# baaivision/Painter

Measured on AMD Instinct MI355X. Metric: images/sec (896x448 pairs) ViT-L fwd+bwd, higher is better.
Workload: dtype bf16; 1 GPU; painter_vit_large_patch16_input896x448 bf16 batch=8/GPU fwd+bwd on 1xMI355X (BASELINE configs[1]); global_batch=8, image=896x448x3 stitched pair, mode=train (DropPath 0.1), parallelism=dp1, rccl_ranks=0, backend=n/a, grad_allreduce=n/a

## Files before the change

include/painter_hip.h:

```cpp
#ifndef PAINTER_HIP_H
#define PAINTER_HIP_H

#include <stdint.h>

#ifdef __cplusplus
extern "C" {
#endif

#ifndef __HIP__
typedef struct ihipStream_t* hipStream_t;
#endif

enum { PA_F32 = 0, PA_BF16 = 1 };
enum {
    PA_EPI_BIAS = 0,
    PA_EPI_BIAS_F32 = 1,
    PA_EPI_BIAS_GELU = 2,
    PA_EPI_BIAS_RESID = 3
};

#define PA_ABI_VERSION 8
int pa_abi_version(void);
int pa_debug_set(int which, int value);
int pa_debug_get(int which);
// ... 5 lines not shown
int pa_linear_fwd_skip(int dtype, int epilogue, const void* x, int64_t ldx, const void* w, const float* bias, void* out, void* out2,
                       int64_t ldo, const float* resid, const float* rowscale, int rows_per_sample, int M, int N, int K,
                       const float* rowskip, int skip_rows_per_sample, hipStream_t stream);
int pa_linear_pixshuf(int dtype, const void* x, int64_t ldx, const void* w , const float* bias,
                      void* out_nhwc, int batch, int Hp, int Wp, int P, int C, int K, hipStream_t stream);
int64_t pa_linear_dgrad_workspace_bytes(int M, int K);
int pa_linear_dgrad(int dtype, const void* dy , int64_t lddy, const void* w ,
                    const void* gelu_aux , void* dx , int64_t lddx, float* dx_colsum,
                    void* workspace, int M, int N, int K, hipStream_t stream);
int pa_linear_dgrad_skip(int dtype, const void* dy, int64_t lddy, const void* w, const void* gelu_aux, void* dx, int64_t lddx, float* dx_colsum,
                         void* workspace, int M, int N, int K, const float* rowskip , int skip_rows_per_sample,
                         hipStream_t stream);
int64_t pa_linear_wgrad_workspace_bytes(int dtype, int M, int N, int K);
int pa_linear_wgrad(int dtype, const void* dy , int64_t lddy, const void* x , int64_t ldx,
                    float* dw , void* workspace, int M, int N, int K, hipStream_t stream);
int64_t pa_colsum_workspace_bytes(int M, int N);
int pa_colsum(int dtype, const void* x , int64_t ld, int M, int N, float* out , void* workspace,
              hipStream_t stream);
int pa_slab_reduce(const float* in, float* out, int64_t n, int nz, int64_t stride, int accumulate, hipStream_t stream);

int pa_layernorm_fwd(int dtype, const float* x, int64_t ldx, const float* gamma, const float* beta, float eps,
                     void* y , int64_t ldy, float* mean, float* rstd,
                     int R, int D, hipStream_t stream);
int64_t pa_layernorm_bwd_workspace_bytes(int R, int D);
int pa_layernorm_bwd(int dtype, const void* dy, int64_t lddy, const float* x, int64_t ldx, const float* mean,
                     const float* rstd, const float* gamma, const float* dres, float* dx, int64_t lddx, void* dxT,
                     int64_t lddxT, const float* rowscale, int rows_per_sample, float* dgamma_dbeta, float* dxT_colsum,
                     void* workspace, int R, int D, hipStream_t stream);
int pa_layernorm_bwd_reduce(const void* workspace, float* dgamma_dbeta, float* dxT_colsum, int with_colsum, int R, int D,
                            hipStream_t stream);
// ... 196 lines not shown
```

painter_amd/_lib.py:

```python
import ctypes
import os
import re

HERE = os.path.dirname(os.path.abspath(__file__))
HEADER = os.path.join(os.path.dirname(HERE), "include", "painter_hip.h")
LIB_PATH = os.environ.get("PAINTER_AMD_LIB") or os.path.join(HERE, "lib", "libpainter_hip.so")

PA_F32, PA_BF16 = 0, 1
EPI_BIAS, EPI_BIAS_F32, EPI_BIAS_GELU, EPI_BIAS_RESID = 0, 1, 2, 3
(KNOB_G256_STAGGER, KNOB_G256_NOSTORE, KNOB_G256_ORDER, KNOB_WGRAD_TARGET, KNOB_G256_SHORT_TILES, KNOB_G256_ILV, KNOB_RELPOS_SPLITS,
 KNOB_ATTN3_FUSE, KNOB_ATTN_LIGHT_LAST, KNOB_CONV_WGRAD_GROUPS, KNOB_LN_BWD_VARIANT, KNOB_G256_PATCH, KNOB_G256_MIXED) = range(13)
KNOB_G256_MIXED_NFULL, KNOB_DROP_SKIP, KNOB_DECODER_ROWS, KNOB_COUNT = 14, 16, 17, 18

_CT = {"int": ctypes.c_int, "int64_t": ctypes.c_int64, "float": ctypes.c_float, "hipStream_t": ctypes.c_void_p}


def parse_header(path=HEADER):
    src = open(path).read()
    src = re.sub(r"/\*.*?\*/", " ", src, flags=re.S)
    src = re.sub(r"//[^\n]*", " ", src)
    protos = {}
    for m in re.finditer(r"\b(int64_t|int)\s+(pa_\w+)\s*\(([^)]*)\)\s*;", src):
        ret, name, args = m.group(1), m.group(2), m.group(3).strip()
        argtypes = []
        if args and args != "void":
            for a in args.split(","):
                a = a.strip()
# ... 47 lines not shown
```

painter_amd/csrc/common.h:

```cpp
#pragma once
#include <hip/hip_runtime.h>
#include <stdint.h>
#include <cstdlib>

typedef __bf16 bf16;
typedef __attribute__((ext_vector_type(8))) __bf16 bf16x8;
typedef __attribute__((ext_vector_type(16))) float f32x16;

#define DEVI __device__ __forceinline__

template <typename T> struct TT;
template <> struct TT<float> {
    static constexpr int EPC = 4;
    static constexpr int BK = 32;
    static constexpr int KSTEPS = 2;
    static constexpr int SPF = 2;
    typedef uint4 Vec4;
};
template <> struct TT<bf16> {
    static constexpr int EPC = 8;
    static constexpr int BK = 64;
    static constexpr int KSTEPS = 4;
    static constexpr int SPF = 1;
    typedef uint2 Vec4;
// ... 69 lines not shown

enum Knob {
    KNOB_G256_STAGGER = 0,
    KNOB_G256_NOSTORE = 1,
    KNOB_G256_ORDER = 2,
    KNOB_WGRAD_TARGET = 3,
    KNOB_G256_SHORT_TILES = 4,
    KNOB_G256_ILV = 5,
    KNOB_RELPOS_SPLITS = 6,
    KNOB_ATTN3_FUSE = 7,
    KNOB_ATTN_LIGHT_LAST = 8,
    KNOB_CONV_WGRAD_GROUPS = 9,
    KNOB_LN_BWD_VARIANT = 10,
    KNOB_G256_PATCH = 11,
    KNOB_G256_MIXED = 12,
    KNOB_FREE_13 = 13,
    KNOB_G256_MIXED_NFULL = 14,
    KNOB_FREE_15 = 15,
    KNOB_DROP_SKIP = 16,
    KNOB_DECODER_ROWS = 17,
    KNOB_COUNT = 18
};
inline int g_knob[KNOB_COUNT] = {};
static inline bool drop_skip_on() {
    static const int env = [] { const char* v = getenv("PAINTER_AMD_DROP_SKIP"); return v ? atoi(v) : 1; }();
    return g_knob[KNOB_DROP_SKIP] == 1 ? false : (g_knob[KNOB_DROP_SKIP] == 2 ? true : env != 0);
}
static inline bool decoder_rows_on() {
    static const int env = [] { const char* v = getenv("PAINTER_AMD_DECODER_ROWS"); return v ? atoi(v) : 1; }();
    return g_knob[KNOB_DECODER_ROWS] == 1 ? false : (g_knob[KNOB_DECODER_ROWS] == 2 ? true : env != 0);
}

inline long long g_attn_counts[6] = {0, 0, 0, 0, 0, 0};

DEVI float gelu_f(float x) { return 0.5f * x * (1.0f + erff(x * 0.70710678118654752f)); }
DEVI float gelu_grad_f(float x) {
    const float cdf = 0.5f * (1.0f + erff(x * 0.70710678118654752f));
    const float pdf = 0.39894228040143268f * __expf(-0.5f * x * x);
    return cdf + x * pdf;
}

// ... 71 lines not shown
```

painter_amd/csrc/gemm.hip:

```cpp
#include <cstdlib>
#include "gemm_engine.h"
#include "gemm256.h"
#include "../../include/painter_hip.h"

template <typename OutT> struct EpiBias {
    OutT* out; size_t ldo; const float* bias; int M, N;
    DEVI void operator()(const f32x16 (&acc)[2][2], int ib, int jb, int lane, int) const {
        foreach_acc(acc, ib, jb, lane, [&](int i, int j, float v) {
            if (i < M && j < N) out[(size_t)i * ldo + j] = from_f<OutT>(v + (bias ? bias[j] : 0.f));
        });
    }
};
constexpr float G8_OFF = 0.13f, G8_SCALE = 255.f / 1.26f, G8_STEP = 1.26f / 255.f;
DEVI uint32_t g8_code(float g) { return min((uint32_t)fmaf(g, G8_SCALE, G8_OFF * G8_SCALE + 0.5f), 255u); }
DEVI float g8_value(uint32_t q) { return fmaf((float)q, G8_STEP, -G8_OFF); }
template <typename T> struct GeluAux { typedef T type; };
template <> struct GeluAux<bf16> { typedef unsigned char type; };
template <typename T> struct EpiBiasGelu {
    typename GeluAux<T>::type* aux; T* act; size_t ld; const float* bias; int M, N;
    DEVI void operator()(const f32x16 (&acc)[2][2], int ib, int jb, int lane, int) const {
        foreach_acc(acc, ib, jb, lane, [&](int i, int j, float v) {
            if (i < M && j < N) {
                const T p = from_f<T>(v + bias[j]);
                if constexpr (std::is_same<T, bf16>::value) {
// ... 487 lines not shown
                                    rowskip, skip_rows_per_sample);
    return linear_dgrad_t<float>((const float*)dy, lddy, (const float*)w, (const float*)gelu_aux, (float*)dx, lddx, dx_colsum, (float*)workspace, M, N, K, st);
}
extern "C" int pa_linear_dgrad(int dtype, const void* dy, int64_t lddy, const void* w, const void* gelu_aux,
                               void* dx, int64_t lddx, float* dx_colsum, void* workspace, int M, int N, int K, hipStream_t st) {
    return pa_linear_dgrad_skip(dtype, dy, lddy, w, gelu_aux, dx, lddx, dx_colsum, workspace, M, N, K, nullptr, 1, st);
}

static bool wgrad_fast(int dtype, int M, int N, int K) {
    return dtype == PA_BF16 && g256::ok(N, K, M, true, true, N, K) && K % 4 == 0 && N % 256 == 0 && K % 256 == 0;
}
static int wgrad_fast_splits(int M, int N, int K) {
    const int tiles = (N / 256) * (K / 256);
    static const int env_target = [] { const char* v = getenv("PA_WGRAD_WGS"); return v ? atoi(v) : 0; }();
    int target = env_target > 0 ? env_target : (g_knob[KNOB_WGRAD_TARGET] > 0 ? g_knob[KNOB_WGRAD_TARGET] : 256);
    if (target < 16) target = 16;
    int s = (target + 3 * tiles / 4) / tiles;
    if (s < 1) s = 1;
    const int ktiles = M / 64;
    if (s > ktiles / 4) s = ktiles / 4 > 0 ? ktiles / 4 : 1;
    return g256::splits_used(M, s);
}
static int wgrad_splits(int M, int N, int K, int bk) {
    const int tiles = ((N + 127) / 128) * ((K + 127) / 128);
    const int nku = (M + bk - 1) / bk;
    int s = (640 + tiles - 1) / tiles;
    if (s > nku) s = nku;
    if (s > 64) s = 64;
    if (s < 1) s = 1;
    return s;
}
extern "C" int64_t pa_linear_wgrad_workspace_bytes(int dtype, int M, int N, int K) {
    if (wgrad_fast(dtype, M, N, K)) {
        const int s = wgrad_fast_splits(M, N, K);
        return s > 1 ? (int64_t)s * N * K * sizeof(float) : 0;
    }
    const int s = wgrad_splits(M, N, K, dtype == PA_BF16 ? 64 : 32);
    return s > 1 ? (int64_t)s * N * K * sizeof(float) : 0;
}
template <typename T>
static int linear_wgrad_t(const T* dy, int64_t lddy, const T* x, int64_t ldx, float* dw, float* ws, int M, int N, int K,
                          hipStream_t st) {
    if constexpr (std::is_same<T, bf16>::value) {
        if (wgrad_fast(PA_BF16, M, N, K) && g256::ok(N, K, M, true, true, lddy, ldx)) {
            const int s = wgrad_fast_splits(M, N, K);
            if (s == 1) return g256::launch<true, true>(dy, lddy, x, ldx, Epi4Slab{dw, (size_t)K, 0, N, K}, N, K, M, 1, st);
            int e = g256::launch<true, true>(dy, lddy, x, ldx, Epi4Slab{ws, (size_t)K, (size_t)N * K, N, K}, N, K, M, s, st);
            if (e) return e;
            return pa_slab_reduce(ws, dw, (int64_t)N * K, s, (int64_t)N * K, 0, st);
        }
    }
    OpT<T> A{dy, (size_t)lddy, N, 0};
    OpT<T> B{x, (size_t)ldx, K, 0};
    const int s = wgrad_splits(M, N, K, TT<T>::BK);
    if (s == 1) return launch_gemm<T, 2, 2>(A, B, EpiSlab{dw, (size_t)K, 0, N, K}, N, K, M, 1, 1, st);
    int e = launch_gemm<T, 2, 2>(A, B, EpiSlab{ws, (size_t)K, (size_t)N * K, N, K}, N, K, M, s, 1, st);
    if (e) return e;
    return pa_slab_reduce(ws, dw, (int64_t)N * K, s, (int64_t)N * K, 0, st);
}
extern "C" int pa_linear_wgrad(int dtype, const void* dy, int64_t lddy, const void* x, int64_t ldx, float* dw,
                               void* workspace, int M, int N, int K, hipStream_t st) {
    if (N % 4 || K % 4) return (int)hipErrorInvalidValue;
    if (dtype == PA_BF16) return linear_wgrad_t<bf16>((const bf16*)dy, lddy, (const bf16*)x, ldx, dw, (float*)workspace, M, N, K, st);
    return linear_wgrad_t<float>((const float*)dy, lddy, (const float*)x, ldx, dw, (float*)workspace, M, N, K, st);
}

extern "C" int pa_fill_dead_rows(void* x, int64_t pitch_bytes, int64_t row_bytes, const int* rowmap, int M, hipStream_t st);
extern "C" int pa_linear_dgrad_live(const void* dy, int64_t lddy, const void* w, void* dx, int64_t lddx, const int* live, const int* rowmap,
                                    const int* count, int M, int N, int K, hipStream_t st) {
    if (live == nullptr || rowmap == nullptr || count == nullptr || M < 8 || K % 8 || lddx % 8) return (int)hipErrorInvalidValue;
    if (!g256::ok(M, K, N, false, true, lddy, K)) return (int)hipErrorInvalidValue;
    int e = pa_fill_dead_rows(dx, lddx * 2, (int64_t)K * 2, rowmap, M, st);
    if (e) return e;
    return g256::launch_live<false, true>((const bf16*)dy, lddy, (const bf16*)w, K, Epi4Scatter{(bf16*)dx, (size_t)lddx, live, count, M, K}, M, K, N, count, st);
}
extern "C" int pa_linear_wgrad_live(const void* dy, int64_t lddy, const void* x, int64_t ldx, float* dw, const int* count, int M, int N, int K,
                                    hipStream_t st) {
    if (count == nullptr || M < 128 || M % 128) return (int)hipErrorInvalidValue;
    if (!wgrad_fast(PA_BF16, M, N, K) || !g256::ok(N, K, M, true, true, lddy, ldx)) return (int)hipErrorInvalidValue;
// ... 13 lines not shown
```

painter_amd/csrc/gemm256.h:

```cpp
#pragma once
#include "common.h"
#include <cstdlib>
#include <type_traits>

namespace g256 {

constexpr int BM = 256, BN = 256, BK = 64, NT = 512;
constexpr int LDS_BYTES = 131072;
typedef __attribute__((address_space(3))) void lds_void;
typedef __attribute__((address_space(1))) const void gbl_cvoid;

DEVI constexpr int unit_off(bool isB, int sub, int stage) { return (isB ? 65536 : 0) + sub * 32768 + stage * 16384; }

template <int N> DEVI void wait_vm() { asm volatile("s_waitcnt vmcnt(%0)" ::"n"(N) : "memory"); }
DEVI void wait_lgkm0() { asm volatile("s_waitcnt lgkmcnt(0)" ::: "memory"); }

template <bool MM, bool IS_A>
DEVI uint32_t src_off(int tid, int j, int sub, int tile0, int rows, uint32_t ld) {
    const int cidx = j * NT + tid;
    if constexpr (!MM) {
        const int u = cidx >> 3, p = cidx & 7;
        const int kc = p ^ ((u >> 1) & 7);
        int row = IS_A ? ((u >> 6) * 128 + sub * 64 + (u & 63)) : ((u >> 5) * 64 + sub * 32 + (u & 31));
        row = min(tile0 + row, rows - 1);
        return ((uint32_t)row * ld + kc * 8) * 2u;
    } else {
        const int k = cidx >> 4, cp = cidx & 15;
        const int c = cp ^ (4 * (k & 3));
        int n = IS_A ? ((c >> 3) * 128 + sub * 64 + (c & 7) * 8) : ((c >> 2) * 64 + sub * 32 + (c & 3) * 8);
        n = min(tile0 + n, rows - 8);
        return ((uint32_t)k * ld + n) * 2u;
    }
}

DEVI const unsigned char* sgpr_ptr(const unsigned char* p) {
    asm volatile("" : "+s"(p));
    return p;
}
DEVI void dma16(const unsigned char* g, unsigned char* l) {
    __builtin_amdgcn_global_load_lds((gbl_cvoid*)g, (lds_void*)l, 16, 0, 0);
}

template <int OFF> DEVI void lds_read128(uint4& d, uint32_t addr) {
    asm volatile("ds_read_b128 %0, %1 offset:%2" : "=v"(d) : "v"(addr), "n"(OFF) : "memory");
}
template <int OFF> DEVI void lds_read64_tr(uint2& d, uint32_t addr) {
    asm volatile("ds_read_b64_tr_b16 %0, %1 offset:%2" : "=v"(d) : "v"(addr), "n"(OFF) : "memory");
}

template <bool MM> struct Frag4;
template <> struct Frag4<false> {
    uint4 q0, q1, q2, q3;
    template <int IMM> DEVI void read(const uint32_t (&base)[4], int) {
// ... 22 lines not shown
    template <int KS> DEVI bf16x8 k() const {
        typedef __attribute__((ext_vector_type(2))) uint32_t u2;
        typedef __attribute__((ext_vector_type(4))) uint32_t u4;
        const uint2 l = KS == 0 ? l0 : KS == 1 ? l1 : KS == 2 ? l2 : l3;
        const uint2 h = KS == 0 ? h0 : KS == 1 ? h1 : KS == 2 ? h2 : h3;
        u2 lv = {l.x, l.y}, hv = {h.x, h.y};
        return __builtin_bit_cast(bf16x8, __builtin_shufflevector(lv, hv, 0, 1, 2, 3));
    }
};

template <class Epi> struct epi_colsum { static constexpr bool value = false; };
template <class Epi, class = void> struct epi_hi_off { static constexpr int value = 4; };
template <class Epi> struct epi_hi_off<Epi, std::void_t<decltype(Epi::HI_OFF)>> { static constexpr int value = Epi::HI_OFF; };
constexpr int BM_SHORT = 224;
constexpr int BM_HALF = 128;
template <bool AMM, bool BMM, int ILV, class Epi, bool SHORT = false, bool MIXED = false, bool SKIP = false, bool LIVE = false>
__global__ __launch_bounds__(NT) void gemm256_kernel(const bf16* __restrict__ Ag, uint32_t lda, const bf16* __restrict__ Bg,
                                                      uint32_t ldb, Epi epi, int M, int N, int ktiles, int ktiles_per_split,
                                                      int tiles_n, int stagger, int order, int nfull, int patch,
                                                      const float* __restrict__ rowskip, int rps, const int* __restrict__ live_count) {
    static_assert(!(LIVE && (SHORT || MIXED || SKIP)), "a device-side count goes with uniform 256-row tiles");
    static_assert(!(SHORT && AMM), "the 224-row tile is built for a K-major A operand");
    static_assert(!(SKIP && AMM), "row tiles are skipped only for a K-major A operand");
    static_assert(!(MIXED && (AMM || SHORT)), "half tiles are built for a K-major A operand and 256-row full tiles");
    constexpr int BMR = SHORT ? BM_SHORT : BM;
    extern __shared__ __attribute__((aligned(1024))) unsigned char smem[];
    const int tid = threadIdx.x, lane = tid & 63;
    if (stagger > 0 && blockIdx.x < 256 && blockIdx.y == 0) {
        const int64_t wait = ((int64_t)stagger * (((blockIdx.x >> 3) * 5) & 15)) >> 4;
        const uint64_t t0 = __builtin_amdgcn_s_memtime();
        while ((int64_t)(__builtin_amdgcn_s_memtime() - t0) < wait) __builtin_amdgcn_s_sleep(16);
    }
    const int wv = __builtin_amdgcn_readfirstlane(tid >> 6);
    const int wr = wv >> 2, wc = wv & 3;

    const bool htile = MIXED && (int)blockIdx.x >= nfull * tiles_n;
    int nwg = MIXED ? (htile ? (int)gridDim.x - nfull * tiles_n : nfull * tiles_n) : (int)gridDim.x;
    if constexpr (LIVE) {
        if constexpr (AMM) {
// ... 70 lines not shown
        if (skipped) {
            const int d = bid - nwg;
            int r = d / tiles_n;
            tn = d - r * tiles_n;
            bool found = false;
            skipped_ranges([&](int a, int b) {
                if (!found && r < b - a) { tm = a + r; found = true; }
                if (!found) r -= b - a;
            });
        } else {
            skipped_ranges([&](int a, int b) { if (tm >= a) tm += b - a; });
        }
    }
    const int i0 = htile ? nfull * BMR + tm * BM_HALF : tm * BMR, j0 = tn * BN;
    const bool blk3 = !(SHORT && wr == 1);
    const int kt0 = split * ktiles_per_split;
    const int nt = min(ktiles - kt0, ktiles_per_split);
    const bool empty = LIVE && AMM && nt == 0;
    uint32_t oa[2][2], ob[2][2];
#pragma unroll
    for (int sub = 0; sub < 2; ++sub)
#pragma unroll
        for (int j = 0; j < 2; ++j) {
            oa[sub][j] = src_off<AMM, true>(tid, j, sub, i0, M, lda);
            ob[sub][j] = src_off<BMM, false>(tid, j, sub, j0, N, ldb);
        }
    const size_t a_step = AMM ? (size_t)BK * lda * 2 : (size_t)BK * 2;
    const size_t b_step = BMM ? (size_t)BK * ldb * 2 : (size_t)BK * 2;
    const unsigned char* abase = reinterpret_cast<const unsigned char*>(Ag) + (size_t)kt0 * a_step;
    const unsigned char* bbase = reinterpret_cast<const unsigned char*>(Bg) + (size_t)kt0 * b_step;
    unsigned char* const dma_dst = smem + wv * 1024;

    auto piece_a = [&](int sub, int stage, int kt, int j) {
// ... 60 lines not shown
    auto pre = [&](auto&& d0, auto&& d1) {
        if constexpr (ILV < 2) d0();
        if constexpr (ILV < 1) d1();
        wait_vm<8 - ILV>();
    };
    auto bar = [&]() {
        __builtin_amdgcn_sched_barrier(0);
        __builtin_amdgcn_s_barrier();
        __builtin_amdgcn_sched_barrier(0);
    };
    auto lwait = [&]() {
        wait_lgkm0();
        __builtin_amdgcn_sched_barrier(0);
    };

    auto tile_body = [&](auto stage_c, int T) {
        constexpr int S = decltype(stage_c)::value;
        const int t1 = min(T + 1, nt - 1), t2 = min(T + 2, nt - 1);
        fa0.template read<unit_off(false, 0, S)>(ra, 0);
        fa1.template read<unit_off(false, 0, S) + (AMM ? 0 : 4096)>(ra, 1);
        fb0.template read<unit_off(true, 0, S) - 65536>(rb, 0);
        {
            auto d0 = [&] { piece_b(1, S ^ 1, t1, 0); };
            auto d1 = [&] { piece_b(1, S ^ 1, t1, 1); };
            pre(d0, d1);
            bar(); lwait();
            mma_quad(0, 0, fb0, d0, d1);
            bar();
        }
        fb1.template read<unit_off(true, 1, S) - 65536>(rb, 0);
        {
            auto d0 = [&] { piece_a(1, S ^ 1, t1, 0); };
            auto d1 = [&] { piece_a(1, S ^ 1, t1, 1); };
// ... 60 lines not shown
    if constexpr (MIXED) {
        if (htile) {
            ran_half = true;
            if (!skipped) {
                piece_a(0, 0, 0, 0); piece_a(1, 0, 0, 0); stage_b(0, 0, 0); stage_b(1, 0, 0);
                wait_vm<0>();
                bar();
                for (int T = 0; T < nt; T += 2) {
                    half_body(I0{}, T);
                    half_body(I1{}, T + 1);
                }
            }
        }
    }
    if (!ran_half && !skipped && !empty) {
        stage_a(0, 0, 0);
        stage_b(0, 0, 0);
        stage_b(1, 0, 0);
        stage_a(1, 0, 0);
        stage_a(0, 1, 1);
        stage_b(0, 1, 1);
        wait_vm<8>();
        bar();
        if (wr == 1) bar();

        for (int T = 0; T < nt; T += 2) {
            tile_body(I0{}, T);
            tile_body(I1{}, T + 1);
        }
    }
    if (wr == 0 && !ran_half && !skipped && !empty) bar();
    wait_vm<0>();

    bar();
    {
        float* stg = reinterpret_cast<float*>(smem + wv * 8704);
        constexpr int HO = epi_hi_off<Epi>::value;
        static_assert(HO == 4 || (HO == 32 && !epi_colsum<Epi>::value), "epilogue column layouts: 8 consecutive, or 4 + 4 at a distance of 32");
        const int lr = lane & 31, g = lane >> 5, rrow = lane >> 3, c0 = (lane & 7) * (HO == 4 ? 8 : 4);
        const int jcol = j0 + wc * 64 + c0;
        const typename Epi::Col col = epi.col(jcol);
        const int rbase = i0 + wr * (htile ? 64 : 128);
        float cs[8] = {0.f, 0.f, 0.f, 0.f, 0.f, 0.f, 0.f, 0.f};
// ... 38 lines not shown
                float v = cs[e];
                v += lane_dpp<0x128>(v);
                v += lane_xor16(v);
                v += lane_xor32(v);
                cs[e] = v;
            }
            if (lane < 8) epi.colsum_out((htile ? nfull + tm : tm) * 2 + wr, jcol, cs);
        }
    }
}

static inline int per_split(int ktiles, int nsplit) {
    int per = (ktiles + nsplit - 1) / nsplit;
    return per + (per & 1);
}
template <bool AMM, bool BMM, int ILV, bool SHORT, class Epi, bool MIXED = false, bool SKIP = false, bool LIVE = false>
static int launch_ilv(const bf16* A, size_t lda, const bf16* B, size_t ldb, Epi epi, int M, int N, int K, int nsplit, hipStream_t st, int nfull = 0,
                      const float* rowskip = nullptr, int rps = 1, const int* live_count = nullptr);
#ifndef G256_ILV_DEFAULT
#define G256_ILV_DEFAULT 2
#endif
static inline bool use_short(int M, int N, int nsplit, bool amm) {
    if (amm || nsplit != 1 || M < BM) return false;
    if (g_knob[KNOB_G256_SHORT_TILES] == 1) return false;
    if (g_knob[KNOB_G256_SHORT_TILES] == 2) return true;
    static const int cost = [] { const char* v = getenv("PA_G256_SHORT_COST"); return v ? atoi(v) : 92; }();
    const int tiles_n = (N + BN - 1) / BN;
    const long t256 = (long)((M + BM - 1) / BM) * tiles_n, t224 = (long)((M + BM_SHORT - 1) / BM_SHORT) * tiles_n;
    const long r256 = (t256 + 255) / 256 * 100, r224 = (t224 + 255) / 256 * cost;
    return r224 < r256;
}
// ... 35 lines not shown
    return launch_ilv<AMM, BMM, G256_ILV_DEFAULT, false>(A, lda, B, ldb, epi, M, N, K, nsplit, st);
#endif
}
template <bool BMM, class Epi>
static int launch_skip(const bf16* A, size_t lda, const bf16* B, size_t ldb, Epi epi, int M, int N, int K, hipStream_t st, const float* rowskip, int rps) {
    if ((M + rps - 1) / rps > 63) return launch<false, BMM>(A, lda, B, ldb, epi, M, N, K, 1, st);
    const TilePlan tp = tile_plan(M, N, 1, false);
    if (tp.mixed) return launch_ilv<false, BMM, G256_ILV_DEFAULT, false, Epi, true, true>(A, lda, B, ldb, epi, M, N, K, 1, st, tp.nfull, rowskip, rps);
    if (tp.is_short) return launch_ilv<false, BMM, G256_ILV_DEFAULT, true, Epi, false, true>(A, lda, B, ldb, epi, M, N, K, 1, st, 0, rowskip, rps);
    return launch_ilv<false, BMM, G256_ILV_DEFAULT, false, Epi, false, true>(A, lda, B, ldb, epi, M, N, K, 1, st, 0, rowskip, rps);
}
template <bool AMM, bool BMM, class Epi>
static int launch_live(const bf16* A, size_t lda, const bf16* B, size_t ldb, Epi epi, int M, int N, int K, const int* live_count, hipStream_t st) {
    return launch_ilv<AMM, BMM, G256_ILV_DEFAULT, false, Epi, false, false, true>(A, lda, B, ldb, epi, M, N, K, 1, st, 0, nullptr, 1, live_count);
}
template <bool AMM, bool BMM, int ILV, bool SHORT, class Epi, bool MIXED, bool SKIP, bool LIVE>
static int launch_ilv(const bf16* A, size_t lda, const bf16* B, size_t ldb, Epi epi, int M, int N, int K, int nsplit, hipStream_t st, int nfull,
                      const float* rowskip, int rps, const int* live_count) {
    auto kern = gemm256_kernel<AMM, BMM, ILV, Epi, SHORT, MIXED, SKIP, LIVE>;
    static bool attr_done = false;
    if (!attr_done) {
        hipError_t e = hipFuncSetAttribute(reinterpret_cast<const void*>(kern), hipFuncAttributeMaxDynamicSharedMemorySize, LDS_BYTES);
        if (e != hipSuccess) return (int)e;
        attr_done = true;
    }
    constexpr int BMR = SHORT ? BM_SHORT : BM;
    static const int env_patch = [] { const char* v = getenv("PA_G256_PATCH"); return v ? atoi(v) : 0; }();
    const int tiles_n = (N + BN - 1) / BN;
    const int tiles_m = MIXED ? nfull + (M - nfull * BMR + BM_HALF - 1) / BM_HALF : (M + BMR - 1) / BMR;
    const int ktiles = K / BK;
    const int per = per_split(ktiles, nsplit);
    const int splits = (ktiles + per - 1) / per;
    if (g_knob[KNOB_G256_NOSTORE]) epi.M = 0;
    PA_LAUNCH(kern, dim3(tiles_m * tiles_n, splits), dim3(NT), LDS_BYTES, st, A, (uint32_t)lda, B, (uint32_t)ldb, epi, M, N,
// ... 24 lines not shown
```

painter_amd/engine.py:

```python
import os
from typing import NamedTuple

import torch

from . import hostmath, ops
from ._lib import EPI_BIAS, EPI_BIAS_F32, EPI_BIAS_RESID, KNOB_RELPOS_SPLITS, KNOB_WGRAD_TARGET


_SIDE_STREAM = os.environ.get("PAINTER_AMD_SIDE_STREAM", "1") != "0"
_DBG_SERIAL = os.environ.get("PAINTER_AMD_DEBUG_SERIAL", "0") == "1"
_DBG_TRACE = os.environ.get("PAINTER_AMD_DEBUG_TRACE", "0") == "1"
_configured = False
WGRAD_SIDE_TARGET = 96
RELPOS_SIDE_SPLITS = 8


def _configure_library():
    global _configured
    if _configured:
        return
    from ._lib import lib
    lib.pa_debug_set(KNOB_RELPOS_SPLITS, RELPOS_SIDE_SPLITS if _SIDE_STREAM else 0)
    lib.pa_debug_set(KNOB_WGRAD_TARGET, WGRAD_SIDE_TARGET if _SIDE_STREAM else 0)
    _configured = True
# ... 113 lines not shown


class _Backward:
    __slots__ = ("P", "S", "sync", "want", "st", "G", "flats", "rc_shape", "dnorm")

    def __init__(self, P, S, sync, want, st):
        self.P, self.S, self.sync, self.want, self.st = P, S, sync, want, st
        self.G = {}
        self.flats = {}
        self.rc_shape = tuple(S.blocks[-1].rcat.shape)
        self.dnorm = None

    def need(self, n):
        return self.want is None or n in self.want

    def param_grads(self, wname, bname, dy, x, bout=None, wgrad=None, colsum=None):
        G = self.G
        do_w, do_b = self.need(wname), bname not in G and self.need(bname)
        if not (do_w or do_b):
            return

        def fn():
            if do_w:
                G[wname] = (wgrad or ops.linear_wgrad)(dy, x)
            if do_b:
                G[bname] = (colsum or ops.colsum)(dy, out=bout)
        self.st.run(fn, dy, x if do_w else None)

    def ready(self, names, flat=None):
        self.st.ready(self.sync, self.G, names, flat=flat)


class HotPath:

    def __init__(self, cfg: HotPathConfig, compute_dtype):
        self.cfg = cfg
        self.T = compute_dtype
        self._M = None
        self._wcache = {}
# ... 269 lines not shown
            fb = X.st.shared(torch.empty((sum(sizes),), dtype=torch.float32, device=X.S.imgs.device))
            X.flats[i] = (fb, dict(zip(("n1", "n2", "qkv", "proj", "fc1", "fc2", "rel"), torch.split(fb, sizes))))
        return X.flats[i]

    def _backward_block(self, X, i, dconcat, dx, dyT_next):
        c, T, P, S, G, st, need = self.cfg, self.T, X.P, X.S, X.G, X.st, X.need
        B, L, D = S.B, c.L, c.D
        dev = S.imgs.device
        tr = self._tr
        pre = "blocks.%d." % i
        b = S.blocks[i]
        S.blocks[i] = None
        R = b.Bc * L
        ds_a, ds_m = (None, None) if S.drop is None else S.drop[i]
        sk_a = None if b.group > 0 else ds_a
        nrp, hd = X.rc_shape
        flat, fl = self.block_flat(X, i)
        del X.flats[i]
        if i in c.taps:
            k = c.taps.index(i)
            tap = S.taps[k]
            dyT = torch.empty((R, D), dtype=T, device=dev)
            dx, gb = ops.layernorm_bwd(dconcat[:, k * D:(k + 1) * D], tap.x, tap.mean, tap.rstd, P["norm.weight"], dres=dx, dx=dx, dxT=dyT,
                                       rowscale=ds_m, rows_per_sample=L, dxT_colsum=fl["fc2"])
            G[pre + "mlp.fc2.bias"] = fl["fc2"]
            if need("norm.weight") or need("norm.bias"):
                X.dnorm = gb if X.dnorm is None else _add_(X.dnorm, gb)
        elif i == c.merge_idx:
            dx, dyT = ops.merge_bwd(T, dx, ds_m, L, B * L, D)
        else:
            dyT = dyT_next
        X.param_grads(pre + "mlp.fc2.weight", pre + "mlp.fc2.bias", dyT, b.act, fl["fc2"])
        tr("%d.dyT" % i, dyT)
        dpre = ops.linear_dgrad(dyT, self.w(pre + "mlp.fc2.weight", P), gelu_aux=b.gaux, colsum_out=fl["fc1"], rowskip=ds_m, rows_per_sample=L)
        G[pre + "mlp.fc1.bias"] = fl["fc1"]
        tr("%d.dpre" % i, dpre)
        X.param_grads(pre + "mlp.fc1.weight", pre + "mlp.fc1.bias", dpre, b.ln2, fl["fc1"])
        dln2 = ops.linear_dgrad(dpre, self.w(pre + "mlp.fc1.weight", P), rowskip=ds_m, rows_per_sample=L)
        tr("%d.dln2" % i, dln2)
        del dpre
        dyA = st.private(dyT)
        lnws, lndone = self.ln_workspace(dev, ops.layernorm_bwd_workspace_bytes(R, D), st.main, st.side)
        dx, fin = ops.layernorm_bwd(dln2, b.x1, b.mean2, b.rstd2, P[pre + "norm2.weight"], dres=dx, dx=dx, dxT=dyA,
                                    rowscale=ds_a, rows_per_sample=L, gb=fl["n2"].view(2, D), dxT_colsum=fl["proj"], defer=True, ws=lnws)
        gb = None
        if need(pre + "norm2.weight") or need(pre + "norm2.bias") or need(pre + "attn.proj.bias"):
            gb = st.run(fin)
            lndone()
            G[pre + "norm2.weight"], G[pre + "norm2.bias"] = gb[0], gb[1]
        G[pre + "attn.proj.bias"] = fl["proj"]
        del dyT
        tr("%d.dx_ln2" % i, dx); tr("%d.dyA" % i, dyA)
        if gb is not None:
            tr("%d.gb2" % i, gb)
        if b.group > 0:
            da = ops.ensemble_resid(torch.zeros_like(dx), dx if ds_a is None else ops.scale_cast(torch.float32, dx, ds_a, L), b.Bc, b.group, L, D)
            dyA = da if T == torch.float32 else ops.cast_bf16(da, out=dyA)
            del da
        X.param_grads(pre + "attn.proj.weight", pre + "attn.proj.bias", dyA, b.ao, fl["proj"])
        dao = ops.linear_dgrad(dyA, self.w(pre + "attn.proj.weight", P), out=dln2, rowskip=sk_a, rows_per_sample=L)
        tr("%d.dao" % i, dao)
        del dyA
        rcatT = self.relpos(pre, P, True)
        dqkv, dG = ops.attn_bwd_core(b.qkv, b.rcat, rcatT, b.ao, dao, b.lse, b.Bc, L, c.heads, c.Hp, c.Wp, c.scale, tables=b.atab, rowskip=sk_a)
        if need(pre + "attn.rel_pos_h") or need(pre + "attn.rel_pos_w"):
            drcat = st.run(lambda: ops.attn_bwd_relpos(dG, b.qkv, nrp, b.Bc, L, c.heads, c.Hp, c.Wp, out=fl["rel"].view(nrp, hd)), dG, b.qkv)
            nh, nw = 2 * c.Hp - 1, 2 * c.Wp - 1
            G[pre + "attn.rel_pos_h"] = drcat[:nh]
            G[pre + "attn.rel_pos_w"] = drcat[nh:nh + nw]
        del dG
        tr("%d.dqkv" % i, dqkv)
        X.param_grads(pre + "attn.qkv.weight", pre + "attn.qkv.bias", dqkv, b.ln1, fl["qkv"])
        dln1 = ops.linear_dgrad(dqkv, self.w(pre + "attn.qkv.weight", P), out=dao, rowskip=sk_a, rows_per_sample=L)
        del dqkv
        nxt = i - 1
        if nxt >= 0 and nxt not in c.taps and nxt != c.merge_idx:
            dyT_next = torch.empty((R, D), dtype=T, device=dev)
        else:
            dyT_next = None
        ds_next = None if (S.drop is None or nxt < 0) else S.drop[nxt][1]
        cs_next = None
        if dyT_next is not None:
            cs_next = self.block_flat(X, nxt)[1]["fc2"]
            G["blocks.%d.mlp.fc2.bias" % nxt] = cs_next
        lnws, lndone = self.ln_workspace(dev, ops.layernorm_bwd_workspace_bytes(R, D), st.main, st.side)
        dx, fin = ops.layernorm_bwd(dln1, b.x, b.mean1, b.rstd1, P[pre + "norm1.weight"], dres=dx, dx=dx, dxT=dyT_next,
                                    rowscale=ds_next if dyT_next is not None else None, rows_per_sample=L, gb=fl["n1"].view(2, D),
# ... 52 lines not shown
```

painter_amd/ops.py:

```python
import torch

from ._lib import (EPI_BIAS, EPI_BIAS_F32, EPI_BIAS_GELU, EPI_BIAS_RESID, KNOB_DECODER_ROWS, KNOB_DROP_SKIP, PA_BF16, PA_F32, check, lib)

_WS = {}


def stream():
    return torch.cuda.current_stream().cuda_stream


def code(dtype):
    if dtype == torch.bfloat16:
        return PA_BF16
    if dtype == torch.float32:
        return PA_F32
    raise TypeError("painter_amd supports float32 / bfloat16 operand types, got %s" % dtype)


def p(t):
    return 0 if t is None else t.data_ptr()


def workspace(nbytes, device, slot=0):
    key = (device, slot, torch.cuda.current_stream(device).cuda_stream)
# ... 103 lines not shown
    _req(dy); _req(w, T)
    if out is None:
        out = torch.empty((M, K), dtype=T, device=dy.device)
    if gelu_aux is not None:
        assert gelu_aux.stride(0) == out.stride(0) and gelu_aux.dtype == gelu_aux_dtype(T), (gelu_aux.dtype, gelu_aux.stride(0), out.stride(0))
    ws = None
    if colsum_out is not None:
        assert colsum_out.shape == (K,) and colsum_out.dtype == torch.float32 and colsum_out.is_contiguous()
        ws = workspace(lib.pa_linear_dgrad_workspace_bytes(M, K), dy.device, slot=2)
    sk, srps = _skip_args(rowskip, rows_per_sample, M)
    check(lib.pa_linear_dgrad_skip(code(T), p(dy), dy.stride(0), p(w), p(gelu_aux), p(out), out.stride(0), p(colsum_out), p(ws), M, N, K,
                                   sk, srps, stream()), "pa_linear_dgrad_skip")
    return out


def linear_wgrad(dy, x, out=None, *, live=None):
    if live is not None:
        lv, count = live
        return linear_wgrad_live(dy, gather_rows(x, lv, count), count, out=out)
    M, N = dy.shape
    K = x.shape[1]
    T = dy.dtype
    _req(dy); _req(x, T)
    if out is None:
        out = torch.empty((N, K), dtype=torch.float32, device=dy.device)
    ws = workspace(lib.pa_linear_wgrad_workspace_bytes(code(T), M, N, K), dy.device)
    check(lib.pa_linear_wgrad(code(T), p(dy), dy.stride(0), p(x), x.stride(0), p(out), p(ws), M, N, K, stream()),
          "pa_linear_wgrad")
    return out


def colsum(x, out=None):
    M, N = x.shape
    if out is None:
        out = torch.empty((N,), dtype=torch.float32, device=x.device)
    ws = workspace(lib.pa_colsum_workspace_bytes(M, N), x.device)
    check(lib.pa_colsum(code(x.dtype), p(x), x.stride(0), M, N, p(out), p(ws), stream()), "pa_colsum")
    return out


def decoder_rows(mode=None):
    return _knob(KNOB_DECODER_ROWS, mode)

# ... 400 lines not shown
```

Baseline: 165.1 images/sec.

## Skip DropPath-dropped sample rows in weight-gradient GEMM K loop

Adds a KSKIP variant of the 256-tile GEMM for weight gradients. It builds a per-split ballot mask of K units (sample rows) whose DropPath scale is zero and iterates only over live units, so no dy×x work is spent on dropped samples. The split assignment also changes from contiguous K chunks to interleaved 2-tile units, and the minimum split target is relaxed. This adds mask bookkeeping and scalar selects in the main loop, and can leave K work unevenly spread across splits.

```diff
diff --git a/include/painter_hip.h b/include/painter_hip.h
--- a/include/painter_hip.h
+++ b/include/painter_hip.h
@@ -43,6 +43,8 @@
 int64_t pa_linear_wgrad_workspace_bytes(int dtype, int M, int N, int K);
 int pa_linear_wgrad(int dtype, const void* dy , int64_t lddy, const void* x , int64_t ldx,
                     float* dw , void* workspace, int M, int N, int K, hipStream_t stream);
+int pa_linear_wgrad_skip(int dtype, const void* dy, int64_t lddy, const void* x, int64_t ldx, float* dw, void* workspace, int M, int N, int K,
+                         const float* rowskip, int skip_rows_per_sample, hipStream_t stream);
 int64_t pa_colsum_workspace_bytes(int M, int N);
 int pa_colsum(int dtype, const void* x , int64_t ld, int M, int N, float* out , void* workspace,
               hipStream_t stream);
diff --git a/painter_amd/_lib.py b/painter_amd/_lib.py
--- a/painter_amd/_lib.py
+++ b/painter_amd/_lib.py
@@ -10,7 +10,7 @@
 EPI_BIAS, EPI_BIAS_F32, EPI_BIAS_GELU, EPI_BIAS_RESID = 0, 1, 2, 3
 (KNOB_G256_STAGGER, KNOB_G256_NOSTORE, KNOB_G256_ORDER, KNOB_WGRAD_TARGET, KNOB_G256_SHORT_TILES, KNOB_G256_ILV, KNOB_RELPOS_SPLITS,
  KNOB_ATTN3_FUSE, KNOB_ATTN_LIGHT_LAST, KNOB_CONV_WGRAD_GROUPS, KNOB_LN_BWD_VARIANT, KNOB_G256_PATCH, KNOB_G256_MIXED) = range(13)
-KNOB_G256_MIXED_NFULL, KNOB_DROP_SKIP, KNOB_DECODER_ROWS, KNOB_COUNT = 14, 16, 17, 18
+KNOB_WGRAD_SKIP, KNOB_G256_MIXED_NFULL, KNOB_DROP_SKIP, KNOB_DECODER_ROWS, KNOB_COUNT = 13, 14, 16, 17, 18
 
 _CT = {"int": ctypes.c_int, "int64_t": ctypes.c_int64, "float": ctypes.c_float, "hipStream_t": ctypes.c_void_p}
 
diff --git a/painter_amd/csrc/common.h b/painter_amd/csrc/common.h
--- a/painter_amd/csrc/common.h
+++ b/painter_amd/csrc/common.h
@@ -107,7 +107,7 @@
     KNOB_LN_BWD_VARIANT = 10,
     KNOB_G256_PATCH = 11,
     KNOB_G256_MIXED = 12,
-    KNOB_FREE_13 = 13,
+    KNOB_WGRAD_SKIP = 13,
     KNOB_G256_MIXED_NFULL = 14,
     KNOB_FREE_15 = 15,
     KNOB_DROP_SKIP = 16,
@@ -118,6 +118,12 @@
 static inline bool drop_skip_on() {
     static const int env = [] { const char* v = getenv("PAINTER_AMD_DROP_SKIP"); return v ? atoi(v) : 1; }();
     return g_knob[KNOB_DROP_SKIP] == 1 ? false : (g_knob[KNOB_DROP_SKIP] == 2 ? true : env != 0);
+}
+static inline bool wgrad_skip_on() {
+    static const int env = [] { const char* v = getenv("PAINTER_AMD_WGRAD_SKIP"); return v ? (atoi(v) != 0 ? 1 : 0) : -1; }();
+    if (g_knob[KNOB_WGRAD_SKIP] == 1) return false;
+    if (g_knob[KNOB_WGRAD_SKIP] == 2) return true;
+    return env >= 0 ? env != 0 : drop_skip_on();
 }
 static inline bool decoder_rows_on() {
     static const int env = [] { const char* v = getenv("PAINTER_AMD_DECODER_ROWS"); return v ? atoi(v) : 1; }();
diff --git a/painter_amd/csrc/gemm.hip b/painter_amd/csrc/gemm.hip
--- a/painter_amd/csrc/gemm.hip
+++ b/painter_amd/csrc/gemm.hip
@@ -525,7 +525,7 @@
     const int tiles = (N / 256) * (K / 256);
     static const int env_target = [] { const char* v = getenv("PA_WGRAD_WGS"); return v ? atoi(v) : 0; }();
     int target = env_target > 0 ? env_target : (g_knob[KNOB_WGRAD_TARGET] > 0 ? g_knob[KNOB_WGRAD_TARGET] : 256);
-    if (target < 16) target = 16;
+    if (target < 1) target = 1;
     int s = (target + 3 * tiles / 4) / tiles;
     if (s < 1) s = 1;
     const int ktiles = M / 64;
@@ -551,10 +551,16 @@
 }
 template <typename T>
 static int linear_wgrad_t(const T* dy, int64_t lddy, const T* x, int64_t ldx, float* dw, float* ws, int M, int N, int K,
-                          hipStream_t st) {
+                          hipStream_t st, const float* rowskip = nullptr, int skip_rps = 1) {
     if constexpr (std::is_same<T, bf16>::value) {
         if (wgrad_fast(PA_BF16, M, N, K) && g256::ok(N, K, M, true, true, lddy, ldx)) {
             const int s = wgrad_fast_splits(M, N, K);
+            const Epi4Slab ep = s == 1 ? Epi4Slab{dw, (size_t)K, 0, N, K} : Epi4Slab{ws, (size_t)K, (size_t)N * K, N, K};
+            if (rowskip != nullptr) {
+                int e = g256::launch_wskip(dy, lddy, x, ldx, ep, N, K, M, s, st, rowskip, skip_rps);
+                if (e || s == 1) return e;
+                return pa_slab_reduce(ws, dw, (int64_t)N * K, s, (int64_t)N * K, 0, st);
+            }
             if (s == 1) return g256::launch<true, true>(dy, lddy, x, ldx, Epi4Slab{dw, (size_t)K, 0, N, K}, N, K, M, 1, st);
             int e = g256::launch<true, true>(dy, lddy, x, ldx, Epi4Slab{ws, (size_t)K, (size_t)N * K, N, K}, N, K, M, s, st);
             if (e) return e;
@@ -569,11 +575,17 @@
     if (e) return e;
     return pa_slab_reduce(ws, dw, (int64_t)N * K, s, (int64_t)N * K, 0, st);
 }
+extern "C" int pa_linear_wgrad_skip(int dtype, const void* dy, int64_t lddy, const void* x, int64_t ldx, float* dw,
+                                    void* workspace, int M, int N, int K, const float* rowskip, int skip_rows_per_sample, hipStream_t st) {
+    if (N % 4 || K % 4) return (int)hipErrorInvalidValue;
+    if (rowskip != nullptr && skip_rows_per_sample < 1) return (int)hipErrorInvalidValue;
+    if (!wgrad_skip_on()) rowskip = nullptr;
+    if (dtype == PA_BF16) return linear_wgrad_t<bf16>((const bf16*)dy, lddy, (const bf16*)x, ldx, dw, (float*)workspace, M, N, K, st, rowskip, skip_rows_per_sample);
+    return linear_wgrad_t<float>((const float*)dy, lddy, (const float*)x, ldx, dw, (float*)workspace, M, N, K, st);
+}
 extern "C" int pa_linear_wgrad(int dtype, const void* dy, int64_t lddy, const void* x, int64_t ldx, float* dw,
                                void* workspace, int M, int N, int K, hipStream_t st) {
-    if (N % 4 || K % 4) return (int)hipErrorInvalidValue;
-    if (dtype == PA_BF16) return linear_wgrad_t<bf16>((const bf16*)dy, lddy, (const bf16*)x, ldx, dw, (float*)workspace, M, N, K, st);
-    return linear_wgrad_t<float>((const float*)dy, lddy, (const float*)x, ldx, dw, (float*)workspace, M, N, K, st);
+    return pa_linear_wgrad_skip(dtype, dy, lddy, x, ldx, dw, workspace, M, N, K, nullptr, 1, st);
 }
 
 extern "C" int pa_fill_dead_rows(void* x, int64_t pitch_bytes, int64_t row_bytes, const int* rowmap, int M, hipStream_t st);
diff --git a/painter_amd/csrc/gemm256.h b/painter_amd/csrc/gemm256.h
--- a/painter_amd/csrc/gemm256.h
+++ b/painter_amd/csrc/gemm256.h
@@ -37,6 +37,11 @@
     asm volatile("" : "+s"(p));
     return p;
 }
+DEVI int sel_nz(unsigned long long m, int a, int b) {
+    int r;
+    asm("s_cmp_lg_u64 %1, 0\n\ts_cselect_b32 %0, %2, %3" : "=s"(r) : "s"(m), "s"(a), "s"(b) : "scc");
+    return r;
+}
 DEVI void dma16(const unsigned char* g, unsigned char* l) {
     __builtin_amdgcn_global_load_lds((gbl_cvoid*)g, (lds_void*)l, 16, 0, 0);
 }
@@ -89,7 +94,7 @@
 template <class Epi> struct epi_hi_off<Epi, std::void_t<decltype(Epi::HI_OFF)>> { static constexpr int value = Epi::HI_OFF; };
 constexpr int BM_SHORT = 224;
 constexpr int BM_HALF = 128;
-template <bool AMM, bool BMM, int ILV, class Epi, bool SHORT = false, bool MIXED = false, bool SKIP = false, bool LIVE = false>
+template <bool AMM, bool BMM, int ILV, class Epi, bool SHORT = false, bool MIXED = false, bool SKIP = false, bool LIVE = false, bool KSKIP = false>
 __global__ __launch_bounds__(NT) void gemm256_kernel(const bf16* __restrict__ Ag, uint32_t lda, const bf16* __restrict__ Bg,
                                                       uint32_t ldb, Epi epi, int M, int N, int ktiles, int ktiles_per_split,
                                                       int tiles_n, int stagger, int order, int nfull, int patch,
@@ -98,6 +103,8 @@
     static_assert(!(SHORT && AMM), "the 224-row tile is built for a K-major A operand");
     static_assert(!(SKIP && AMM), "row tiles are skipped only for a K-major A operand");
     static_assert(!(MIXED && (AMM || SHORT)), "half tiles are built for a K-major A operand and 256-row full tiles");
+    static_assert(!KSKIP || (AMM && BMM && !LIVE && !SKIP), "K units are skipped only in the weight gradient (both operands M-major)");
+    constexpr bool ILEAVE = AMM && BMM && !LIVE;
     constexpr int BMR = SHORT ? BM_SHORT : BM;
     extern __shared__ __attribute__((aligned(1024))) unsigned char smem[];
     const int tid = threadIdx.x, lane = tid & 63;
@@ -198,9 +205,21 @@
     }
     const int i0 = htile ? nfull * BMR + tm * BM_HALF : tm * BMR, j0 = tn * BN;
     const bool blk3 = !(SHORT && wr == 1);
-    const int kt0 = split * ktiles_per_split;
-    const int nt = min(ktiles - kt0, ktiles_per_split);
-    const bool empty = LIVE && AMM && nt == 0;
+    const int nsp = (int)gridDim.y;
+    const int kt0 = ILEAVE ? 0 : split * ktiles_per_split;
+    int nt = ILEAVE ? 2 * (((ktiles >> 1) - split + nsp - 1) / nsp) : min(ktiles - kt0, ktiles_per_split);
+    unsigned long long lmask = 0;
+    if constexpr (KSKIP) {
+        const int rows = ktiles * BK, ns = (rows + rps - 1) / rps;
+        const float fv = lane < ns ? rowskip[lane] : 1.f;
+        const unsigned long long dm = __ballot(fv == 0.f);
+        const int r0 = min((split + lane * nsp) * 128, rows - 128);
+        const int sa = r0 / rps, sb = (r0 + 127) / rps;
+        const unsigned long long range = ((2ull << sb) - 1ull) & ~((1ull << sa) - 1ull);
+        lmask = __ballot(2 * lane < nt && (dm & range) != range);
+        nt = 2 * __builtin_popcountll(lmask);
+    }
+    const bool empty = ((LIVE && AMM) || KSKIP) && nt == 0;
     uint32_t oa[2][2], ob[2][2];
 #pragma unroll
     for (int sub = 0; sub < 2; ++sub)
@@ -291,9 +310,8 @@
         __builtin_amdgcn_sched_barrier(0);
     };
 
-    auto tile_body = [&](auto stage_c, int T) {
+    auto tile_body = [&](auto stage_c, int t1, int t2) {
         constexpr int S = decltype(stage_c)::value;
-        const int t1 = min(T + 1, nt - 1), t2 = min(T + 2, nt - 1);
         fa0.template read<unit_off(false, 0, S)>(ra, 0);
         fa1.template read<unit_off(false, 0, S) + (AMM ? 0 : 4096)>(ra, 1);
         fb0.template read<unit_off(true, 0, S) - 65536>(rb, 0);
@@ -384,19 +402,53 @@
         }
     }
     if (!ran_half && !skipped && !empty) {
-        stage_a(0, 0, 0);
-        stage_b(0, 0, 0);
-        stage_b(1, 0, 0);
-        stage_a(1, 0, 0);
-        stage_a(0, 1, 1);
-        stage_b(0, 1, 1);
+        int cur = 0, n0 = 0, n1 = 0, left = 0;
+        auto next_unit = [&]() {
+            cur = n0;
+            if constexpr (KSKIP) {
+                const int nx = 2 * (split + __builtin_ctzll(lmask | (1ull << 63)) * nsp);
+                n0 = sel_nz(lmask, nx, cur + 1);
+                n1 = sel_nz(lmask, nx + 1, cur + 1);
+                lmask &= lmask - 1;
+            } else {
+                const bool has = left > 0;
+                const int nx = cur + 2 * nsp;
+                left -= has ? 1 : 0;
+                n0 = has ? nx : cur + 1;
+                n1 = has ? nx + 1 : cur + 1;
+            }
+        };
+        if constexpr (ILEAVE) {
+            if constexpr (KSKIP) {
+                n0 = 2 * (split + __builtin_ctzll(lmask) * nsp);
+                lmask &= lmask - 1;
+            } else {
+                n0 = 2 * split;
+                left = (nt >> 1) - 1;
+            }
+            next_unit();
+        }
+        stage_a(0, 0, cur);
+        stage_b(0, 0, cur);
+        stage_b(1, 0, cur);
+        stage_a(1, 0, cur);
+        stage_a(0, 1, cur + 1);
+        stage_b(0, 1, cur + 1);
         wait_vm<8>();
         bar();
         if (wr == 1) bar();
 
-        for (int T = 0; T < nt; T += 2) {
-            tile_body(I0{}, T);
-            tile_body(I1{}, T + 1);
+        if constexpr (!ILEAVE) {
+            for (int T = 0; T < nt; T += 2) {
+                tile_body(I0{}, min(T + 1, nt - 1), min(T + 2, nt - 1));
+                tile_body(I1{}, min(T + 2, nt - 1), min(T + 3, nt - 1));
+            }
+        } else {
+            for (int T = 0; T < nt; T += 2) {
+                tile_body(I0{}, cur + 1, n0);
+                tile_body(I1{}, n0, n1);
+                next_unit();
+            }
         }
     }
     if (wr == 0 && !ran_half && !skipped && !empty) bar();
@@ -465,7 +517,7 @@
     int per = (ktiles + nsplit - 1) / nsplit;
     return per + (per & 1);
 }
-template <bool AMM, bool BMM, int ILV, bool SHORT, class Epi, bool MIXED = false, bool SKIP = false, bool LIVE = false>
+template <bool AMM, bool BMM, int ILV, bool SHORT, class Epi, bool MIXED = false, bool SKIP = false, bool LIVE = false, bool KSKIP = false>
 static int launch_ilv(const bf16* A, size_t lda, const bf16* B, size_t ldb, Epi epi, int M, int N, int K, int nsplit, hipStream_t st, int nfull = 0,
                       const float* rowskip = nullptr, int rps = 1, const int* live_count = nullptr);
 #ifndef G256_ILV_DEFAULT
@@ -531,10 +583,17 @@
 static int launch_live(const bf16* A, size_t lda, const bf16* B, size_t ldb, Epi epi, int M, int N, int K, const int* live_count, hipStream_t st) {
     return launch_ilv<AMM, BMM, G256_ILV_DEFAULT, false, Epi, false, false, true>(A, lda, B, ldb, epi, M, N, K, 1, st, 0, nullptr, 1, live_count);
 }
-template <bool AMM, bool BMM, int ILV, bool SHORT, class Epi, bool MIXED, bool SKIP, bool LIVE>
+static inline int splits_used(int K, int nsplit);
+template <class Epi>
+static int launch_wskip(const bf16* A, size_t lda, const bf16* B, size_t ldb, Epi epi, int M, int N, int K, int nsplit, hipStream_t st, const float* rowskip, int rps) {
+    const int units = K / (2 * BK), splits = splits_used(K, nsplit);
+    if ((K + rps - 1) / rps > 63 || (units + splits - 1) / splits > 64) return launch<true, true>(A, lda, B, ldb, epi, M, N, K, nsplit, st);
+    return launch_ilv<true, true, G256_ILV_DEFAULT, false, Epi, false, false, false, true>(A, lda, B, ldb, epi, M, N, K, nsplit, st, 0, rowskip, rps);
+}
+template <bool AMM, bool BMM, int ILV, bool SHORT, class Epi, bool MIXED, bool SKIP, bool LIVE, bool KSKIP>
 static int launch_ilv(const bf16* A, size_t lda, const bf16* B, size_t ldb, Epi epi, int M, int N, int K, int nsplit, hipStream_t st, int nfull,
                       const float* rowskip, int rps, const int* live_count) {
-    auto kern = gemm256_kernel<AMM, BMM, ILV, Epi, SHORT, MIXED, SKIP, LIVE>;
+    auto kern = gemm256_kernel<AMM, BMM, ILV, Epi, SHORT, MIXED, SKIP, LIVE, KSKIP>;
     static bool attr_done = false;
     if (!attr_done) {
         hipError_t e = hipFuncSetAttribute(reinterpret_cast<const void*>(kern), hipFuncAttributeMaxDynamicSharedMemorySize, LDS_BYTES);
diff --git a/painter_amd/engine.py b/painter_amd/engine.py
--- a/painter_amd/engine.py
+++ b/painter_amd/engine.py
@@ -151,7 +151,7 @@
     def need(self, n):
         return self.want is None or n in self.want
 
-    def param_grads(self, wname, bname, dy, x, bout=None, wgrad=None, colsum=None):
+    def param_grads(self, wname, bname, dy, x, bout=None, wgrad=None, colsum=None, rowskip=None, rows_per_sample=1):
         G = self.G
         do_w, do_b = self.need(wname), bname not in G and self.need(bname)
         if not (do_w or do_b):
@@ -159,7 +159,7 @@
 
         def fn():
             if do_w:
-                G[wname] = (wgrad or ops.linear_wgrad)(dy, x)
+                G[wname] = wgrad(dy, x) if wgrad else ops.linear_wgrad(dy, x, rowskip=rowskip, rows_per_sample=rows_per_sample)
             if do_b:
                 G[bname] = (colsum or ops.colsum)(dy, out=bout)
         self.st.run(fn, dy, x if do_w else None)
@@ -459,6 +459,7 @@
         R = b.Bc * L
         ds_a, ds_m = (None, None) if S.drop is None else S.drop[i]
         sk_a = None if b.group > 0 else ds_a
+        wk_m, wk_a = (None, None) if T == torch.float32 else (ds_m, sk_a)
         nrp, hd = X.rc_shape
         flat, fl = self.block_flat(X, i)
         del X.flats[i]
@@ -475,12 +476,12 @@
             dx, dyT = ops.merge_bwd(T, dx, ds_m, L, B * L, D)
         else:
             dyT = dyT_next
-        X.param_grads(pre + "mlp.fc2.weight", pre + "mlp.fc2.bias", dyT, b.act, fl["fc2"])
+        X.param_grads(pre + "mlp.fc2.weight", pre + "mlp.fc2.bias", dyT, b.act, fl["fc2"], rowskip=wk_m, rows_per_sample=L)
         tr("%d.dyT" % i, dyT)
         dpre = ops.linear_dgrad(dyT, self.w(pre + "mlp.fc2.weight", P), gelu_aux=b.gaux, colsum_out=fl["fc1"], rowskip=ds_m, rows_per_sample=L)
         G[pre + "mlp.fc1.bias"] = fl["fc1"]
         tr("%d.dpre" % i, dpre)
-        X.param_grads(pre + "mlp.fc1.weight", pre + "mlp.fc1.bias", dpre, b.ln2, fl["fc1"])
+        X.param_grads(pre + "mlp.fc1.weight", pre + "mlp.fc1.bias", dpre, b.ln2, fl["fc1"], rowskip=wk_m, rows_per_sample=L)
         dln2 = ops.linear_dgrad(dpre, self.w(pre + "mlp.fc1.weight", P), rowskip=ds_m, rows_per_sample=L)
         tr("%d.dln2" % i, dln2)
         del dpre
@@ -502,7 +503,7 @@
             da = ops.ensemble_resid(torch.zeros_like(dx), dx if ds_a is None else ops.scale_cast(torch.float32, dx, ds_a, L), b.Bc, b.group, L, D)
             dyA = da if T == torch.float32 else ops.cast_bf16(da, out=dyA)
             del da
-        X.param_grads(pre + "attn.proj.weight", pre + "attn.proj.bias", dyA, b.ao, fl["proj"])
+        X.param_grads(pre + "attn.proj.weight", pre + "attn.proj.bias", dyA, b.ao, fl["proj"], rowskip=wk_a, rows_per_sample=L)
         dao = ops.linear_dgrad(dyA, self.w(pre + "attn.proj.weight", P), out=dln2, rowskip=sk_a, rows_per_sample=L)
         tr("%d.dao" % i, dao)
         del dyA
@@ -515,7 +516,7 @@
             G[pre + "attn.rel_pos_w"] = drcat[nh:nh + nw]
         del dG
         tr("%d.dqkv" % i, dqkv)
-        X.param_grads(pre + "attn.qkv.weight", pre + "attn.qkv.bias", dqkv, b.ln1, fl["qkv"])
+        X.param_grads(pre + "attn.qkv.weight", pre + "attn.qkv.bias", dqkv, b.ln1, fl["qkv"], rowskip=wk_a, rows_per_sample=L)
         dln1 = ops.linear_dgrad(dqkv, self.w(pre + "attn.qkv.weight", P), out=dao, rowskip=sk_a, rows_per_sample=L)
         del dqkv
         nxt = i - 1
diff --git a/painter_amd/ops.py b/painter_amd/ops.py
--- a/painter_amd/ops.py
+++ b/painter_amd/ops.py
@@ -1,6 +1,6 @@
 import torch
 
-from ._lib import (EPI_BIAS, EPI_BIAS_F32, EPI_BIAS_GELU, EPI_BIAS_RESID, KNOB_DECODER_ROWS, KNOB_DROP_SKIP, PA_BF16, PA_F32, check, lib)
+from ._lib import (EPI_BIAS, EPI_BIAS_F32, EPI_BIAS_GELU, EPI_BIAS_RESID, KNOB_DECODER_ROWS, KNOB_DROP_SKIP, KNOB_WGRAD_SKIP, PA_BF16, PA_F32, check, lib)
 
 _WS = {}
 
@@ -141,8 +141,13 @@
     return out
 
 
-def linear_wgrad(dy, x, out=None, *, live=None):
+def wgrad_skip(mode=None):
+    return _knob(KNOB_WGRAD_SKIP, mode)
+
+
+def linear_wgrad(dy, x, out=None, *, live=None, rowskip=None, rows_per_sample=1):
     if live is not None:
+        assert rowskip is None
         lv, count = live
         return linear_wgrad_live(dy, gather_rows(x, lv, count), count, out=out)
     M, N = dy.shape
@@ -152,8 +157,9 @@
     if out is None:
         out = torch.empty((N, K), dtype=torch.float32, device=dy.device)
     ws = workspace(lib.pa_linear_wgrad_workspace_bytes(code(T), M, N, K), dy.device)
-    check(lib.pa_linear_wgrad(code(T), p(dy), dy.stride(0), p(x), x.stride(0), p(out), p(ws), M, N, K, stream()),
-          "pa_linear_wgrad")
+    sk, srps = _skip_args(rowskip, rows_per_sample, M)
+    check(lib.pa_linear_wgrad_skip(code(T), p(dy), dy.stride(0), p(x), x.stride(0), p(out), p(ws), M, N, K, sk, srps, stream()),
+          "pa_linear_wgrad_skip")
     return out
 
 
```

New measurement: 165.1 images/sec. About the same (-0.0%).
